# pk17r/online_3d_reconstruction

Measured on AMD Instinct MI355X. Metric: frames_per_sec, higher is better.
Workload: dtype f32; 1 GPU; synthetic 1280x720 dense stereo, jump_pixels 1, 200 frames/GPU, voxel_size 0.05, min_points_per_voxel 1, SOR off, frames resident in HBM (BASELINE.json configs[1]); frames_per_gpu=200, rows=720, cols=1280, jump_pixels=1, parallelism=frame-sharded x1

## Files before the change

### online_3d_reconstruction_amd/csrc/kernels/bookkeeping.inc

```

__global__ void k_minmax_init(float* mm, int64_t mm_stride, int slot, uint32_t* n_kp, int frames)
{
    const int i = blockIdx.x * blockDim.x + threadIdx.x;
    if (i < frames * 6) {
        const int f = i / 6, a = i % 6;
        mm[((int64_t)f * mm_stride + slot) * 6 + a] = (a < 3) ? __builtin_inff() : -__builtin_inff();
    }
    if (n_kp && i < frames) n_kp[i] = 0;
}
__global__ void k_set_counts(uint32_t* n_dev, uint32_t value, int frames)
{
    const int i = blockIdx.x * blockDim.x + threadIdx.x;
    if (i < frames) n_dev[i] = value;
}

__device__ __forceinline__ int64_t scan_row_len(const VoxelGeom* __restrict__ geom, int f, int pass, int n_tiles,
                                                int64_t L)
{
    if (!geom) return L;
    const VoxelGeom g = geom[f];
    if (g.overflow || pass >= (int)g.passes) return 0;
    return (int64_t)geom_bins(g) * n_tiles;
}
__device__ __forceinline__ int scan_live_tiles(const VoxelGeom* __restrict__ geom, int f, int n_tiles)
{
    if (!geom) return n_tiles;
    const int64_t live = ((int64_t)geom[f].n + kSortTile - 1) / kSortTile;
    return live < n_tiles ? (int)live : n_tiles;
}
__global__ __launch_bounds__(1024) void k_scan_rows(uint32_t* __restrict__ data, int64_t L_in, int64_t row_stride,
                                                    uint32_t* __restrict__ totals, const uint32_t* __restrict__ add,
                                                    const VoxelGeom* __restrict__ geom, int pass, int n_tiles,
                                                    int chunked)
{
    __shared__ uint32_t lds[1024 / 64 + 1];
    uint32_t* row = data + (int64_t)blockIdx.x * row_stride;
    int64_t L = scan_row_len(geom, blockIdx.x, pass, n_tiles, L_in);
    if (chunked) L = (L + 4095) / 4096;
    if (L == 0 && !totals) return;
    const int64_t chunk = (L + 1023) / 1024;
    const int64_t b = (int64_t)threadIdx.x * chunk;
    const int64_t e = (b + chunk < L) ? b + chunk : L;
    const bool tiles = geom != nullptr && !chunked;
    const int live = tiles ? scan_live_tiles(geom, blockIdx.x, n_tiles) : 0;
    uint32_t s = 0;
    {
        int t = tiles ? (int)(b % n_tiles) : 0;
        for (int64_t i = b; i < e; ++i) {
            if (!tiles || t < live) s += row[i];
            if (tiles && ++t == n_tiles) t = 0;
        }
    }
    uint32_t total;
    uint32_t run = block_excl_scan_u32<16>(s, lds, total);
    {
        int t = tiles ? (int)(b % n_tiles) : 0;
        for (int64_t i = b; i < e; ++i) {
            const uint32_t v = (!tiles || t < live) ? row[i] : 0u;
            row[i] = run;
            run += v;
            if (tiles && ++t == n_tiles) t = 0;
        }
    }
    if (totals && threadIdx.x == 0) totals[blockIdx.x] = total + (add ? add[blockIdx.x] : 0u);
}

__global__ __launch_bounds__(1024) void k_scan_hist_tm(uint32_t* __restrict__ hist, const VoxelGeom* __restrict__ geom, int pass,
                                                       int n_tiles, int all_live)
{
    extern __shared__ uint32_t tm_row[];
    __shared__ uint32_t lds[1024 / 64 + 1];
    const int f = blockIdx.x;
    const VoxelGeom g = geom[f];
// ... 24 lines not shown
            const uint32_t v = tm_row[t * (kMaxRadix + 1) + d];
            tm_row[t * (kMaxRadix + 1) + d] = run;
            run += v;
            if (++t == n_tiles) t = 0, ++d;
        }
    }
    __syncthreads();
    for (int i = threadIdx.x; i < words; i += 1024)
        if ((i & (kMaxRadix - 1)) < bins) row[i] = tm_row[(i >> kMaxRadixBits) * (kMaxRadix + 1) + (i & (kMaxRadix - 1))];
}

constexpr int kScanChunk = 4096;
__global__ __launch_bounds__(256) void k_scan_chunk_sums(const uint32_t* __restrict__ data, int64_t L_in,
                                                         int64_t row_stride, int n_chunks,
                                                         uint32_t* __restrict__ partial,
                                                         const VoxelGeom* __restrict__ geom, int pass, int n_tiles)
{
    __shared__ uint32_t lds[4];
    const int64_t L = scan_row_len(geom, blockIdx.y, pass, n_tiles, L_in);
    if ((int64_t)blockIdx.x * kScanChunk >= L) return;
    const uint32_t* row = data + (int64_t)blockIdx.y * row_stride;
    const int64_t b = (int64_t)blockIdx.x * kScanChunk + (int64_t)threadIdx.x * 16;
    const int live = scan_live_tiles(geom, blockIdx.y, n_tiles);
    int t = geom ? (int)(b % n_tiles) : 0;
    uint32_t s = 0;
#pragma unroll
    for (int k = 0; k < 16; ++k) {
        if (b + k < L && (!geom || t < live)) s += row[b + k];
        if (geom && ++t == n_tiles) t = 0;
    }
    s = wave_sum_u32(s);
    if ((threadIdx.x & 63) == 0) lds[threadIdx.x >> 6] = s;
    __syncthreads();
    if (threadIdx.x == 0) partial[(int64_t)blockIdx.y * n_chunks + blockIdx.x] = lds[0] + lds[1] + lds[2] + lds[3];
}
__global__ __launch_bounds__(256) void k_scan_chunk_apply(uint32_t* __restrict__ data, int64_t L_in, int64_t row_stride,
                                                          int n_chunks, const uint32_t* __restrict__ partial_scanned,
                                                          const VoxelGeom* __restrict__ geom, int pass, int n_tiles)
{
    __shared__ uint32_t lds[5];
    const int64_t L = scan_row_len(geom, blockIdx.y, pass, n_tiles, L_in);
    if ((int64_t)blockIdx.x * kScanChunk >= L) return;
    uint32_t* row = data + (int64_t)blockIdx.y * row_stride;
    const int64_t b = (int64_t)blockIdx.x * kScanChunk + (int64_t)threadIdx.x * 16;
    const int live = scan_live_tiles(geom, blockIdx.y, n_tiles);
    int t = geom ? (int)(b % n_tiles) : 0;
    uint32_t v[16];
    uint32_t s = 0;
#pragma unroll
    for (int k = 0; k < 16; ++k) {
        v[k] = (b + k < L && (!geom || t < live)) ? row[b + k] : 0u;
        s += v[k];
        if (geom && ++t == n_tiles) t = 0;
    }
    uint32_t total;
    uint32_t run = block_excl_scan_u32<4>(s, lds, total) + partial_scanned[(int64_t)blockIdx.y * n_chunks + blockIdx.x];
#pragma unroll
    for (int k = 0; k < 16; ++k) {
        if (b + k < L) row[b + k] = run;
        run += v[k];
    }
}

__global__ __launch_bounds__(kPtThreads) void k_points_minmax(const o3dr_point* __restrict__ in, int64_t in_fstride,
                                                              const uint32_t* __restrict__ n_dev, int64_t mm_stride,
                                                              float* __restrict__ mm)
// ... 26 lines not shown
```

### online_3d_reconstruction_amd/csrc/kernels/voxel_index.inc

```

__device__ __forceinline__ uint64_t geom_cells(const VoxelGeom& g)
{
    return (uint64_t)(uint32_t)g.div_b[0] * (uint64_t)(uint32_t)g.div_b[1] * (uint64_t)(uint32_t)g.div_b[2];
}
__device__ __forceinline__ void sort_plan(VoxelGeom& g, uint64_t cells)
{
    uint32_t nbits = 32;
    if (cells <= (1ull << 32)) nbits = cells > 1 ? 64u - (uint32_t)__clzll((long long)(cells - 1)) : 1u;
    if (nbits < 1) nbits = 1;
    g.passes = (nbits + kMaxRadixBits - 1) / kMaxRadixBits;
    g.bpp = (nbits + g.passes - 1) / g.passes;
}

__device__ __forceinline__ VoxelGeom voxel_geom_of(const float mn_in[3], const float mx_in[3], const float leaf[3], float z_offset,
                                                   uint32_t n)
{
    VoxelGeom g;
    g.n = n;
    g.overflow = 0;
    g.passes = 0;
    g.bpp = 1;
    g.buf0 = 0;
    g.grouped = 0;
    float mn[3], mx[3];
// ... 142 lines not shown
        if (lane == 0 && i > 0 && i < g.n) prev = group_coord_of(src[i - 1], g.inv, z_offset, cell);
        const bool head = i < g.n && (i == 0 || group_differs(gc, prev));
        c += head ? 1u : 0u;
        const unsigned long long hm = __ballot(head);
        if (lane < 16)
            head_bits[(int64_t)tile * 256 + k * 64 + (threadIdx.x >> 6) * 16 + lane] = (uint8_t)((hm >> (4 * lane)) & 15ull);
    }
    c = wave_sum_u32(c);
    if (lane == 0) lds[threadIdx.x >> 6] = c;
    __syncthreads();
    if (threadIdx.x == 0) seg_cnt[tile] = lds[0] + lds[1] + lds[2] + lds[3];
}
__global__ __launch_bounds__(256) void k_head_counts(const uint8_t* __restrict__ head_bits, const VoxelGeom* __restrict__ geom,
                                                     int n_tiles, uint32_t* __restrict__ seg_cnt)
{
    const int tile = blockIdx.x * 4 + (threadIdx.x >> 6), lane = threadIdx.x & 63;
    const VoxelGeom g = geom[0];
    if (g.overflow || tile >= n_tiles) return;
    const int64_t base = (int64_t)tile * kSegTile;
    uint32_t c = 0;
    if (base < g.n) {
        uint32_t bits = reinterpret_cast<const uint32_t*>(head_bits + (int64_t)tile * 256)[lane];
        const int64_t i0 = base + lane * 16;
#pragma unroll
        for (int q = 0; q < 16; ++q)
            if (i0 + q >= (int64_t)g.n) bits &= ~(1u << ((q >> 2) * 8 + (q & 3)));
        c = (uint32_t)__popc(bits & 0x0f0f0f0fu);
    }
    c = wave_sum_u32(c);
    if (lane == 0) seg_cnt[tile] = c;
}
```

### online_3d_reconstruction_amd/csrc/kernels/voxel_runs.inc

```



constexpr int kHeadWaves = 4;
__device__ __forceinline__ uint32_t run_heads_tile(const uint32_t* __restrict__ k, int f, int64_t cap, int64_t n, int tile, int lane)
{
    const int64_t i0 = (int64_t)tile * kSegTile + lane * 16;
    uint32_t kk[16];
    if (((((int64_t)f * cap) & 3) == 0) && i0 + 15 < n) {
#pragma unroll
        for (int q = 0; q < 4; ++q) {
            const uint4 v = *reinterpret_cast<const uint4*>(k + i0 + 4 * q);
            kk[4 * q] = v.x; kk[4 * q + 1] = v.y; kk[4 * q + 2] = v.z; kk[4 * q + 3] = v.w;
        }
    } else {
#pragma unroll
        for (int q = 0; q < 16; ++q) kk[q] = (i0 + q < n) ? k[i0 + q] : 0u;
    }
    uint32_t prev = (uint32_t)wave_shr1_i32((int32_t)kk[15]);
    if (lane == 0) prev = (i0 > 0 && i0 < n) ? k[i0 - 1] : 0u;
    uint32_t bits = 0;
#pragma unroll
    for (int q = 0; q < 16; ++q) {
        const int64_t i = i0 + q;
        if (i < n && (i == 0 || kk[q] != (q ? kk[q - 1] : prev))) bits |= 1u << ((q >> 2) * 8 + (q & 3));
// ... 145 lines not shown
}

__global__ __launch_bounds__(256) void k_frame_offsets(const VoxelGeom* __restrict__ geom, const uint32_t* __restrict__ n_vox,
                                                       const uint32_t* __restrict__ n_keep,
                                                       const uint32_t* __restrict__ n_grp, int frames, int passthrough,
                                                       uint32_t* __restrict__ n_out, uint64_t* __restrict__ out_off,
                                                       CloudCounters* __restrict__ cc, SortStats* __restrict__ stats,
                                                       const VoxelGeom* __restrict__ sort_geom, int side_heads)
{
    __shared__ uint32_t scan_lds[5];
    __shared__ unsigned long long acc[6];
    if (threadIdx.x < 6) acc[threadIdx.x] = 0;
    __syncthreads();
    const uint64_t base = cc->count;
    uint64_t carry = 0;
    for (int f0 = 0; f0 < frames; f0 += 256) {
        const int f = f0 + threadIdx.x;
        uint32_t m = 0;
        if (f < frames) {
            const VoxelGeom g = geom[f];
            if (passthrough) {
                m = g.n;
            } else if (g.overflow) {
                m = g.n;
                atomicOr(&acc[3], (unsigned long long)O3DR_STATUS_VOXEL_OVERFLOW);
            } else {
                m = (n_grp && sort_geom[f].grouped) ? n_grp[f] : (n_keep ? n_keep[f] : n_vox[f]);
                atomicAdd(&acc[0], (unsigned long long)sort_geom[f].n * g.passes);
                atomicAdd(&acc[5], (unsigned long long)sort_geom[f].n);
                if (side_heads && g.passes != 0u) atomicAdd(&acc[4], (unsigned long long)sort_geom[f].n);
                atomicAdd(&acc[1], (unsigned long long)g.n);
                atomicAdd(&acc[2], (unsigned long long)m);
            }
        }
        uint32_t total;
        const uint32_t excl = block_excl_scan_u32<4>(m, scan_lds, total);
        if (f < frames) {
            n_out[f] = m;
            out_off[f] = base + carry + excl;
        }
        carry += total;
    }
    __syncthreads();
    if (threadIdx.x == 0) {
        cc->count = base + carry;
        cc->status |= (uint32_t)acc[3];
        if (stats) {
            stats->sort_record_passes += acc[0];
            stats->voxel_points_in += acc[1];
            stats->voxel_points_out += acc[2];
            stats->sort_records += acc[5];
            stats->side_head_records += acc[4];
        }
    }
}

// ... 437 lines not shown
```

### online_3d_reconstruction_amd/csrc/o3dr_api.hip

```cpp
#include <dlfcn.h>
#include <stdio.h>
#include <stdlib.h>
#include <string.h>

#include <algorithm>
#include <cfloat>
#include <chrono>
#include <cmath>
#include <condition_variable>
#include <mutex>
#include <string>
#include <vector>

#include <rccl/rccl.h>

#include "../../include/o3dr_testing.h"
#include "o3dr_device.h"
#include "o3dr_image_stack.h"
#include "o3dr_profile.h"

using namespace o3dr;

static thread_local std::string g_err;
static int fail(int code, const char* what)
// ... 44 lines not shown
    Workspace ws;
    size_t ws_elems = 0;
    size_t ws_pts_elems = 0;
    int ws_frames = 0;
    size_t ws_emit_tiles = 0, ws_sort_tiles = 0, ws_seg_tiles = 0, ws_mm_floats = 0;
    DevBuf ws_block, ws_pts_block, ws_grid_block, ws_sor_block;
    int64_t ws_grid_cap = 0, ws_sor_cap = 0;
    int ws_grid_frames = 0, ws_sor_frames = 0;

    o3dr_point* cloud_big = nullptr;
    int64_t cloud_cap = 0;
    o3dr_point* cloud_alt = nullptr;
    int64_t cloud_alt_cap = 0;
    int64_t cloud_ub = 0;
    bool cloud_n_exact = true;
    float* cloud_box = nullptr;
    bool cloud_box_valid = false;
    uint32_t* cloud_heads = nullptr;
    int64_t cloud_heads_cap = 0;
    bool cloud_heads_valid = false;
    float cloud_heads_leaf[3] = {0.f, 0.f, 0.f};
    float cloud_heads_zo = 0.f;
    int cloud_box_enable = 1;
    CloudCounters* cc_big = nullptr;
    CloudCounters* cc_tmp = nullptr;
    CloudCounters* cc_host = nullptr;
    CloudCounters* cc_host_dev = nullptr;
    uint8_t* small_host = nullptr;
    uint32_t* n_host = nullptr;
    uint8_t* misc_dev = nullptr;
// ... 643 lines not shown
    }
    int zero(o3dr_ctx* c)
    {
        if (frames) HIPCHK(hipMemsetAsync(dev, 0, frames * words * sizeof(unsigned long long), c->stream));
        return O3DR_OK;
    }
    unsigned long long* of_frame(size_t f) const { return dev ? dev + f * words : nullptr; }
    int copy_back(o3dr_ctx* c)
    {
        host.resize(frames * words);
        if (frames) HIPCHK(hipMemcpyAsync(host.data(), dev, host.size() * sizeof(unsigned long long), hipMemcpyDeviceToHost, c->stream));
        return O3DR_OK;
    }
};

static int read_counters(o3dr_ctx* c, const CloudCounters* dev, CloudCounters* host, const CloudCounters* dev2 = nullptr,
                         CloudCounters* host2 = nullptr)
{
    HIPCHK(hipMemcpyAsync(c->cc_host, dev, sizeof(CloudCounters), hipMemcpyDeviceToHost, c->stream));
    if (dev2) HIPCHK(hipMemcpyAsync(c->cc_host + 1, dev2, sizeof(CloudCounters), hipMemcpyDeviceToHost, c->stream));
    HIPCHK(hipStreamSynchronize(c->stream));
    *host = *c->cc_host;
    if (dev2) {
        *host2 = c->cc_host[1];
        if (dev2 == c->cc_big) {
            c->cloud_ub = (int64_t)host2->count;
            c->cloud_n_exact = true;
        }
    }
    if (dev == c->cc_big) {
        c->cloud_ub = (int64_t)host->count;
        c->cloud_n_exact = true;
    }
    if ((host->status | (dev2 ? host2->status : 0u)) & O3DR_STATUS_INTERNAL)
        return fail(O3DR_ERR_INTERNAL, "a device-side gather guard tripped (record or point id outside its cloud); results are invalid");
    return O3DR_OK;
}

static int zero_counters(o3dr_ctx* c, CloudCounters* dev)
{
    HIPCHK(hipMemsetAsync(dev, 0, sizeof(CloudCounters), c->stream));
    return O3DR_OK;
}

static int bilateral_prepare(o3dr_ctx* c, int d, double sigma_color, double sigma_space)
{
    if (sigma_color <= 0) sigma_color = 1;
// ... 558 lines not shown
    for (int a = 0; a < 3; ++a) v.cloud_heads.inv[a] = 1.0f / leaf[a];
    v.cloud_heads.z_offset = zo;
}
static const uint8_t* heads_for_merge(o3dr_ctx* c, const float leaf[3], float zo)
{
    if (!c->cloud_heads_valid || !c->cloud_heads) return nullptr;
    if (leaf[0] != c->cloud_heads_leaf[0] || leaf[1] != c->cloud_heads_leaf[1] || leaf[2] != c->cloud_heads_leaf[2] ||
        zo != c->cloud_heads_zo)
        return nullptr;
    return reinterpret_cast<const uint8_t*>(c->cloud_heads);
}

extern "C" int o3dr_cloud_big_reset(o3dr_ctx* c)
{
    CTX_ENTER(c);
    ++c->cloud_gen;
    CHK(zero_counters(c, c->cc_big));
    CHK(cloud_box_clear(c));
    c->cloud_ub = 0;
    c->cloud_n_exact = true;
    return O3DR_OK;
}

extern "C" int o3dr_cloud_big_size(o3dr_ctx* c, int64_t* n, uint32_t* status)
{
    if (n) *n = 0;
    CTX_ENTER(c);
    CloudCounters cc;
    CHK(read_counters(c, c->cc_big, &cc));
    c->cloud_ub = (int64_t)cc.count;
    if (n) *n = (int64_t)cc.count;
    if (status) *status = cc.status;
    return O3DR_OK;
}

extern "C" int o3dr_cloud_big_read(o3dr_ctx* c, o3dr_point* out, int64_t out_capacity, int64_t* n_out, int32_t mem)
{
    if (n_out) *n_out = 0;
    CTX_ENTER(c);
    if (!n_out) return fail(O3DR_ERR_INVALID_ARG, "n_out is NULL");
    CloudCounters cc;
    CHK(read_counters(c, c->cc_big, &cc));
    const int64_t n = (int64_t)cc.count;
    if (n > out_capacity) return fail(O3DR_ERR_CAPACITY, "output buffer too small");
    if (n > 0) {
// ... 12 lines not shown
    if (n < 0 || (n > 0 && !pts)) return fail(O3DR_ERR_INVALID_ARG, "bad arguments");
    if (n == 0) return O3DR_OK;
    if (n >= (int64_t)0xffffffffLL) return fail(O3DR_ERR_INVALID_ARG, "more than 2^32-1 points in one append");
    CHK(cloud_make_room(c, n));
    const void* src;
    CHK(stage_in(c, c->st_in, pts, (size_t)n * sizeof(o3dr_point), mem, &src));
    CHK(ws_ensure(c, 1, 1, false));
    launch_set_counts(&c->prof, c->stream, c->ws.n_valid, (uint32_t)n, 1);
    const float unit_leaf[3] = {1.f, 1.f, 1.f};
    VoxelArgs v = voxel_args((const o3dr_point*)src, 0, c->ws.n_valid, 1, n, unit_leaf);
    v.out_base = c->cloud_big;
    v.cc = c->cc_big;
    v.passthrough = 1;
    c->cloud_box_valid = false;
    c->cloud_heads_valid = false;
    launch_voxel_grid(&c->prof, c->stream, c->ws, v);
    HIPCHK(hipGetLastError());
    c->cloud_ub += n;
    if (mem == O3DR_MEM_HOST) HIPCHK(hipStreamSynchronize(c->stream));
    return O3DR_OK;
}

extern "C" int o3dr_cloud_big_transform(o3dr_ctx* c, const float T[16])
{
    CTX_ENTER(c);
    if (!T) return fail(O3DR_ERR_INVALID_ARG, "T is NULL");
    CloudCounters cc;
    CHK(read_counters(c, c->cc_big, &cc));
    ++c->cloud_gen;
    launch_transform(&c->prof, c->stream, c->cloud_big, (int64_t)cc.count, T, c->cloud_big);
    HIPCHK(hipGetLastError());
    c->cloud_box_valid = false;
    c->cloud_heads_valid = false;
    return O3DR_OK;
}

static int accumulate_impl(o3dr_ctx* c, const uint8_t* disp, int64_t disp_frame_stride, int64_t disp_pitch,
                           const uint8_t* bgr, int64_t bgr_frame_stride, int64_t bgr_pitch, int32_t rows, int32_t cols,
                           const float* poses, int32_t n_frames, const float* kp_xy, const int64_t* kp_offsets, int32_t mem)
{
    CTX_ENTER(c);
    if (!c->has_Q) return fail(O3DR_ERR_NOT_CONFIGURED, "o3dr_set_camera has not been called");
    if (n_frames < 0 || (n_frames > 0 && !poses)) return fail(O3DR_ERR_INVALID_ARG, "bad frame list");
    if (mem != O3DR_MEM_HOST && mem != O3DR_MEM_DEVICE) return fail(O3DR_ERR_INVALID_ARG, "bad mem kind");
// ... 99 lines not shown
            launch_reproject(&c->prof, c->stream, a, nb, c->ws.pts, c->ws.tile_cnt, c->ws.n_kp, c->ws.n_valid, c->ws.mm,
                             c->ws.scan_partial);
        VoxelArgs v = voxel_args(c->ws.pts, cap, c->ws.n_valid, nb, cap, leaf, zo, mp);
        v.keys_ready = fused ? 1 : 0;
        v.emit_tiles = emit_tiles;
        v.cloud_box = c->cloud_box_valid ? c->cloud_box : nullptr;
        heads_for_append(c, v);
        v.out_base = c->cloud_big;
        v.cc = c->cc_big;
        v.passthrough = c->params.dont_downsample ? 1 : 0;
        v.mm_used = a.n_tiles + 1;
        v.stats = c->stats_dev;
        v.test_corrupt = c->test_corrupt;
        c->test_corrupt = 0;
        if (with_sor) CHK(sor_in_front(c, v, false));
        launch_voxel_grid(&c->prof, c->stream, c->ws, v);
        HIPCHK(hipGetLastError());
        c->cloud_ub += (int64_t)nb * cap;
        c->cloud_n_exact = false;
        if (streaming) HIPCHK(hipEventRecord(c->ev_done[slot], c->stream));
    }
    if (streaming) HIPCHK(hipStreamSynchronize(c->stream));
    return O3DR_OK;
}

extern "C" int o3dr_accumulate_frames(o3dr_ctx* c, const uint8_t* disp, int64_t disp_frame_stride, int64_t disp_pitch,
                                      const uint8_t* bgr, int64_t bgr_frame_stride, int64_t bgr_pitch, int32_t rows,
                                      int32_t cols, const float* poses, int32_t n_frames, int32_t mem)
{
    return accumulate_impl(c, disp, disp_frame_stride, disp_pitch, bgr, bgr_frame_stride, bgr_pitch, rows, cols, poses, n_frames,
// ... 346 lines not shown
    return O3DR_OK;
}
extern "C" int o3dr_cloud_big_recv_buffer(o3dr_ctx* c, int64_t n_points, void** ptr)
{
    CTX_ENTER(c);
    if (!ptr || n_points < 0) return fail(O3DR_ERR_INVALID_ARG, "bad arguments");
    CHK(alt_reserve(c, n_points > 0 ? n_points : 1));
    *ptr = c->cloud_alt;
    return O3DR_OK;
}
extern "C" int o3dr_cloud_big_adopt(o3dr_ctx* c, int64_t n_points)
{
    CTX_ENTER(c);
    if (n_points < 0 || n_points > c->cloud_alt_cap) return fail(O3DR_ERR_INVALID_ARG, "more points than the receive buffer holds");
    if (n_points >= (int64_t)0xffffffffLL) return fail(O3DR_ERR_INVALID_ARG, "cloud_big exceeds 2^32-1 points");
    ++c->cloud_gen;
    launch_set_cloud_count(c->stream, c->cc_big, (uint64_t)n_points);
    HIPCHK(hipGetLastError());
    swap_clouds(c);
    c->cloud_box_valid = false;
    c->cloud_heads_valid = false;
    c->cloud_ub = n_points;
    c->cloud_n_exact = true;
    return O3DR_OK;
}

extern "C" int o3dr_cloud_big_header_dev(o3dr_ctx* c, void* hdr_dev)
{
    CTX_ENTER(c);
    if (!hdr_dev) return fail(O3DR_ERR_INVALID_ARG, "hdr_dev is NULL");
    const float* box = c->cloud_box;
// ... 27 lines not shown

extern "C" int o3dr_cloud_big_partition_dev(o3dr_ctx* c, const void* hdrs_dev, int32_t n_hdrs, int32_t n_parts, int64_t* counts_dev)
{
    CTX_ENTER(c);
    if (!hdrs_dev || !counts_dev || n_hdrs < 1 || n_parts < 1 || n_parts > kMaxRadix)
        return fail(O3DR_ERR_INVALID_ARG, "bad arguments (1 <= n_parts <= 128)");
    HIPCHK(hipMemsetAsync(counts_dev, 0, sizeof(int64_t) * ((size_t)n_parts + 1), c->stream));
    const int64_t ub = c->cloud_ub;
    if (ub == 0 || !c->cloud_big) return O3DR_OK;
    if (ub >= (int64_t)0xffffffffLL) return fail(O3DR_ERR_INVALID_ARG, "cloud_big exceeds 2^32-1 points");
    CHK(ws_ensure(c, 1, ub, false));
    CHK(alt_reserve(c, ub));
    o3dr_point* nb = c->cloud_alt;
    launch_count_from_cc(c->stream, c->cc_big, c->ws.n_valid);
    const VoxelArgs v = slice_args(c, ub);
    ++c->cloud_gen;
    launch_partition(&c->prof, c->stream, c->ws, v, n_parts, nb, (uint64_t*)counts_dev, (uint32_t*)(counts_dev + n_parts), hdrs_dev, n_hdrs);
    if (hipGetLastError() != hipSuccess) return fail(O3DR_ERR_HIP, "partition launch failed");
    swap_clouds(c);
    c->cloud_heads_valid = false;
    return O3DR_OK;
}

extern "C" int o3dr_cloud_big_slice_counts_dev(o3dr_ctx* c, const void* hdrs_dev, int32_t n_hdrs, int32_t n_parts, int64_t* counts_dev)
{
    CTX_ENTER(c);
    if (!hdrs_dev || !counts_dev || n_hdrs < 1 || n_parts < 1 || n_parts > kMaxRadix)
        return fail(O3DR_ERR_INVALID_ARG, "bad arguments (1 <= n_parts <= 128)");
    c->place_ub = -1;
    HIPCHK(hipMemsetAsync(counts_dev, 0, sizeof(int64_t) * ((size_t)n_parts + 1), c->stream));
    const int64_t ub = c->cloud_ub;
// ... 20 lines not shown
    if (!counts || n_parts < 1 || n_parts > kMaxRadix || own_part < 0 || own_part >= n_parts || n_before < 0 || n_after < 0)
        return fail(O3DR_ERR_INVALID_ARG, "bad arguments");
    if (c->place_ub < 0 || c->place_parts != n_parts) return fail(O3DR_ERR_INVALID_ARG, "o3dr_cloud_big_slice_counts_dev must run first, for the same slices");
    int64_t n_local = 0;
    for (int p = 0; p < n_parts; ++p) {
        if (counts[p] < 0) return fail(O3DR_ERR_INVALID_ARG, "negative slice size");
        n_local += counts[p];
    }
    if (n_local > c->place_ub) return fail(O3DR_ERR_INVALID_ARG, "slice sizes above the cloud's size");
    const int64_t own = counts[own_part], send_start = n_before + own + n_after, total = send_start + (n_local - own);
    if (send_offset) *send_offset = send_start;
    const int64_t cap_counted = c->place_ub;
    c->place_ub = -1;
    if (n_before == 0 && n_after == 0 && own == n_local) return O3DR_OK;
    if (total >= (int64_t)0xffffffffLL) return fail(O3DR_ERR_INVALID_ARG, "the exchange buffer exceeds 2^32-1 points");
    ++c->cloud_gen;
    CHK(alt_reserve(c, total > 0 ? total : 1));
    int64_t* sh = (int64_t*)(c->misc_host + 2560);
    int64_t nat = 0, out_off = send_start;
    for (int p = 0; p < n_parts; ++p) {
        if (p == own_part) {
            sh[p] = n_before - nat;
        } else {
            sh[p] = out_off - nat;
            out_off += counts[p];
        }
        nat += counts[p];
    }
    HIPCHK(hipMemcpyAsync(c->misc_dev + 2560, sh, sizeof(int64_t) * (size_t)n_parts, hipMemcpyHostToDevice, c->stream));
    if (n_local > 0) {
        const VoxelArgs v = slice_args(c, cap_counted);
// ... 1 lines not shown
        if (hipGetLastError() != hipSuccess) return fail(O3DR_ERR_HIP, "slice placement launch failed");
    }
    swap_clouds(c);
    c->cloud_box_valid = false;
    c->cloud_heads_valid = false;
    c->cloud_ub = total;
    c->cloud_n_exact = false;
    return O3DR_OK;
}

extern "C" int o3dr_cloud_big_set_size(o3dr_ctx* c, int64_t n_points)
{
    CTX_ENTER(c);
    if (n_points < 0 || n_points > c->cloud_cap) return fail(O3DR_ERR_INVALID_ARG, "more points than the cloud buffer holds");
    if (n_points >= (int64_t)0xffffffffLL) return fail(O3DR_ERR_INVALID_ARG, "cloud_big exceeds 2^32-1 points");
    ++c->cloud_gen;
    launch_set_cloud_count(c->stream, c->cc_big, (uint64_t)n_points);
    HIPCHK(hipGetLastError());
    c->cloud_box_valid = false;
    c->cloud_heads_valid = false;
    c->cloud_ub = n_points;
    c->cloud_n_exact = true;
    return O3DR_OK;
}

extern "C" int o3dr_cloud_big_raw_view(o3dr_ctx* c, void** ptr, int64_t* capacity_points)
{
    CTX_ENTER(c);
    if (!ptr || !capacity_points) return fail(O3DR_ERR_INVALID_ARG, "ptr / capacity is NULL");
    *ptr = c->cloud_big;
    *capacity_points = c->cloud_cap;
// ... 38 lines not shown
    for (int p = 0; p < n_parts; ++p) counts[p] = 0;
    CloudCounters cc;
    CHK(read_counters(c, c->cc_big, &cc));
    const int64_t n = (int64_t)cc.count;
    c->cloud_ub = n;
    if (n == 0) return O3DR_OK;
    if (n >= (int64_t)0xffffffffLL) return fail(O3DR_ERR_INVALID_ARG, "cloud_big exceeds 2^32-1 points");
    CHK(ws_ensure(c, 1, n, false));
    CHK(alt_reserve(c, n));
    o3dr_point* nb = c->cloud_alt;
    launch_set_counts(&c->prof, c->stream, c->ws.n_valid, (uint32_t)n, 1);
    CHK(put_bbox(c, gmin, gmax));
    const VoxelArgs v = slice_args(c, n);
    uint32_t* ovf_dev = (uint32_t*)(c->misc_dev + 32);
    uint64_t* cnt_dev = (uint64_t*)(c->misc_dev + 64);
    ++c->cloud_gen;
    launch_partition(&c->prof, c->stream, c->ws, v, n_parts, nb, cnt_dev, ovf_dev);
    if (hipGetLastError() != hipSuccess) return fail(O3DR_ERR_HIP, "partition launch failed");
    HIPCHK(hipMemcpyAsync(c->misc_host, c->misc_dev, 64 + 8 * (size_t)n_parts, hipMemcpyDeviceToHost, c->stream));
    HIPCHK(hipStreamSynchronize(c->stream));
    swap_clouds(c);
    c->cloud_heads_valid = false;
    const uint32_t ovf = *(const uint32_t*)(c->misc_host + 32);
    const uint64_t* hc = (const uint64_t*)(c->misc_host + 64);
    for (int p = 0; p < n_parts; ++p) counts[p] = (int64_t)hc[p];
    if (status) *status = ovf ? O3DR_STATUS_VOXEL_OVERFLOW : 0u;
    return O3DR_OK;
}

struct RcclApi {
    void* handle = nullptr;
// ... 175 lines not shown
    if (own != O3DR_OK) {
        snprintf(buf, sizeof buf, "%s [every rank left the exchange]", own_msg.c_str());
        g_err = buf;
        return own;
    }
    snprintf(buf, sizeof buf, "rank %d failed with code %lld: every rank left the exchange together", first_rank, (long long)first_code);
    g_err = buf;
    return O3DR_ERR_PEER;
}

static int merge_partitioned_impl(o3dr_ctx* c, Transport& T, int32_t gather_result, o3dr_point* out, int64_t out_capacity,
                                  int64_t* n_out, int64_t* n_total, uint32_t* status, int32_t mem)
{
    const int W = T.W, rank = T.rank;
    if (W < 1 || W > kMaxRadix || rank < 0 || rank >= W) return fail(O3DR_ERR_INVALID_ARG, "communicators of 1..128 ranks are supported");
    ++c->cloud_gen;
    const size_t RW = (size_t)W + kRowExtra;
    const size_t o_hdr = 0, o_hdrs = 32, o_row = o_hdrs + 32 * (size_t)W, o_mat = o_row + 8 * RW;
    const size_t total_bytes = o_mat + 8 * (size_t)W * RW;
    CHK(dev_ensure(c, c->st_xchg, total_bytes));
    if (c->xchg_host_cap < total_bytes) {
        if (c->xchg_host) (void)hipHostFree(c->xchg_host);
        c->xchg_host = nullptr;
        c->xchg_host_cap = 0;
        if (hipHostMalloc((void**)&c->xchg_host, total_bytes, hipHostMallocDefault) != hipSuccess) return fail(O3DR_ERR_ALLOC, "hipHostMalloc failed");
        c->xchg_host_cap = total_bytes;
    }
    memset(c->xchg_stats, 0, sizeof c->xchg_stats);
    char* d = (char*)c->st_xchg.p;
    struct Hdr {
        float mn[3], mx[3];
// ... 3433 lines not shown
```

### online_3d_reconstruction_amd/csrc/o3dr_kernels.hip

```cpp
#include <string.h>

#include "o3dr_device.h"
#include "o3dr_profile.h"

namespace o3dr {

#include "kernels/util.inc"
#include "kernels/reproject.inc"
#include "kernels/bookkeeping.inc"
#include "kernels/prepass.inc"
#include "kernels/voxel_index.inc"
#include "kernels/radix_sort.inc"
#include "kernels/voxel_runs.inc"
#include "kernels/incremental.inc"
#include "kernels/multigpu.inc"
#include "kernels/sor.inc"
#include "kernels/small.inc"
#include "kernels/rigid_core.inc"
#include "kernels/nn.inc"
#include "kernels/mls.inc"
#include "kernels/cluster.inc"
#include "kernels/cell_order.inc"
#include "kernels/plane.inc"
#include "kernels/mesh.inc"
// ... 4 lines not shown
#include "kernels/plane_disparity.inc"
#include "kernels/orb.inc"
#include "kernels/stereo.inc"
#include "kernels/disparity_filter.inc"
#include "kernels/multiview.inc"
#include "kernels/segment_image.inc"
#include "kernels/rectify.inc"
#include "kernels/pose_chain.inc"
#include "kernels/ransac.inc"
#include "kernels/pose_graph.inc"

static inline int cdiv64(int64_t a, int64_t b) { return (int)((a + b - 1) / b); }

static void launch_scan(hipStream_t s, uint32_t* data, int64_t L, int64_t row_stride, int frames, uint32_t* totals,
                        const uint32_t* add, uint32_t* partial, const VoxelGeom* geom = nullptr, int pass = 0,
                        int n_tiles = 0)
{
    if (L <= 4 * kScanChunk) {
        k_scan_rows<<<frames, 1024, 0, s>>>(data, L, row_stride, totals, add, geom, pass, n_tiles, 0);
        return;
    }
    const int n_chunks = cdiv64(L, kScanChunk);
    k_scan_chunk_sums<<<dim3(n_chunks, frames), 256, 0, s>>>(data, L, row_stride, n_chunks, partial, geom, pass, n_tiles);
    k_scan_rows<<<frames, 1024, 0, s>>>(partial, L, n_chunks, totals, add, geom, pass, n_tiles, 1);
    k_scan_chunk_apply<<<dim3(n_chunks, frames), 256, 0, s>>>(data, L, row_stride, n_chunks, partial, geom, pass, n_tiles);
}

void launch_minmax_init(Profiler* pf, hipStream_t s, float* mm, int64_t mm_stride, int slot, uint32_t* n_kp, int frames)
{
    ProfScope ps(pf, O3DR_K_OTHER, s);
    k_minmax_init<<<cdiv64(frames * 6, 256), 256, 0, s>>>(mm, mm_stride, slot, n_kp, frames);
}

void launch_set_counts(Profiler* pf, hipStream_t s, uint32_t* n_dev, uint32_t value, int frames)
{
    ProfScope ps(pf, O3DR_K_OTHER, s);
    k_set_counts<<<cdiv64(frames, 256), 256, 0, s>>>(n_dev, value, frames);
}

void launch_small_frame(Profiler* pf, hipStream_t s, const ReprojectArgs& a, const float* kp_xy, int n_kp, int downsample,
// ... 139 lines not shown
}

static void group_run_front(Profiler* pf, hipStream_t s, Workspace& ws, const SortShape& sh, const o3dr_point* in, float z_offset,
                            const uint8_t* rec_heads, int64_t shift_first, int64_t shift_n, int force_runs, int64_t grp_slots)
{
    const int F = sh.frames, n_seg_tiles = sh.n_seg_tiles;
    const uint8_t* hb = rec_heads && shift_n <= 0 ? rec_heads : ws.head_bits;
    {
        ProfScope ps(pf, O3DR_K_KEYGEN, s);
        if (rec_heads && shift_n > 0) {
            const int64_t bytes = (int64_t)n_seg_tiles * 256;
            k_inc_heads_shift<<<cdiv64(bytes, 256), 256, 0, s>>>(rec_heads, (uint64_t)shift_first, (uint64_t)shift_n, ws.head_bits,
                                                                 (uint64_t)bytes);
        }
        if (rec_heads)
            k_head_counts<<<cdiv64(n_seg_tiles, 4), 256, 0, s>>>(hb, ws.geom, n_seg_tiles, ws.seg_cnt);
        else
            k_group_heads<<<n_seg_tiles, 256, 0, s>>>(in, ws.geom, z_offset, n_seg_tiles, ws.seg_cnt, ws.head_bits);
    }
    {
        ProfScope ps(pf, O3DR_K_OTHER, s);
        launch_scan(s, ws.seg_cnt, n_seg_tiles, n_seg_tiles, F, ws.n_runs, nullptr, ws.scan_partial);
    }
    {
        ProfScope ps(pf, O3DR_K_SEGMENT, s);
        k_run_geom<<<cdiv64(F, 64), 64, 0, s>>>(ws.geom, ws.n_runs, F, ws.geom_runs, force_runs, grp_slots);
        k_run_starts<<<dim3(cdiv64(n_seg_tiles, kStartWaves), F), kStartWaves * kWave, 0, s>>>(
            ws.keys[0], ws.keys[1], sh.cap, ws.geom, n_seg_tiles, ws.seg_cnt, ws.n_runs, ws.run_start, 0, ws.keys[1], ws.geom_runs, in,
            z_offset, hb);
    }
}
// ... 140 lines not shown
            {
                ProfScope ps(pf, O3DR_K_OTHER, s);
                launch_scan(s, ws.seg_cnt, n_seg_tiles, n_seg_tiles, F, ws.n_out, nullptr, ws.scan_partial);
            }
            {
                ProfScope ps(pf, O3DR_K_SEGMENT, s);
                k_keep_write<<<sgrid, 256, 0, s>>>(ws.seg_start, cap, sort_geom, ws.n_vox, v.min_points, n_seg_tiles, ws.seg_cnt,
                                                  ws.keep_idx);
            }
            n_keep = ws.n_out;
        }
        if (v.test_corrupt) corrupt_payload(s, ws, sort_geom);
    }
    if (cap > 0 && use_runs) {
        {
            ProfScope ps(pf, O3DR_K_OTHER, s);
            (void)hipMemsetAsync(ws.grp_cnt, 0, sizeof(uint32_t) * (size_t)(max_groups + 1), s);
        }
        {
            ProfScope ps(pf, O3DR_K_CENTROID_RUNS, s);
            int64_t nwg = cdiv64(max_groups < cap ? max_groups : cap, kGroupWaves);
            if (nwg > 16384) nwg = 16384;
            if (nwg < 1) nwg = 1;
            k_centroid_groups<<<(int)nwg, kGroupWaves * kWave, 0, s>>>(
                v.in, ws.keys[0], ws.keys[1], ws.vals[0], ws.vals[1], ws.seg_start, ws.run_start, ws.geom_runs, ws.geom, ws.n_vox,
                v.z_offset, v.min_points, reinterpret_cast<uint4*>(ws.pts), grp_slots, ws.grp_cnt, v.cc);
        }
        {
            ProfScope ps(pf, O3DR_K_OTHER, s);
            launch_scan(s, ws.grp_cnt, max_groups + 1, max_groups + 1, 1, ws.n_grp_out, nullptr, ws.scan_partial);
        }
    }
    {
        ProfScope ps(pf, O3DR_K_OTHER, s);
        k_frame_offsets<<<1, 256, 0, s>>>(ws.geom, ws.n_vox, n_keep, use_runs ? ws.n_grp_out : nullptr, F, v.passthrough,
                                          ws.n_out, ws.out_off, v.cc, v.stats, sort_geom,
                                          (!use_runs && ws.side && !v.passthrough && cap > 0) ? 1 : 0);
    }
    const int nbx = cdiv64(cap, kPtThreads);
    if (cap > 0 && use_runs) {
        ProfScope ps(pf, O3DR_K_CENTROID_RUNS, s);
        int64_t nwg = cdiv64(cap, 256);
        if (nwg > 8192) nwg = 8192;
        k_group_compact<<<(int)nwg, 256, 0, s>>>(v.in, ws.geom_runs, ws.geom, ws.n_vox, ws.grp_cnt,
                                                reinterpret_cast<const uint4*>(ws.pts), ws.out_off, v.z_offset, v.out_base);
// ... 841 lines not shown
```

Measured before the change: 36040 frames/s.

## Bound group-count scan by live length, drop memset, densify head counts, cache size

The group-count scan now takes a per-frame live length (n_vox), so it scans only live+1 entries and treats the rest as zero. This lets the grp_cnt memset be removed, relying on the centroid kernel to write every live slot. k_head_counts now handles four tiles per wave using 16-byte loads and a 16-lane shuffle reduction, and k_frame_offsets reduces its stat atomics across each wave before issuing them. The host cloud-size query reuses the last read counters instead of doing a device read while the cloud is unchanged. The risk is stale grp_cnt entries if any live slot goes unwritten, and a stale cached size if some write path misses the invalidation.

After: 36450 frames/s (median of 6 runs). 1.1% higher.

```diff
diff --git a/online_3d_reconstruction_amd/csrc/kernels/bookkeeping.inc b/online_3d_reconstruction_amd/csrc/kernels/bookkeeping.inc
--- a/online_3d_reconstruction_amd/csrc/kernels/bookkeeping.inc
+++ b/online_3d_reconstruction_amd/csrc/kernels/bookkeeping.inc
@@ -15,8 +15,9 @@
 }
 
 __device__ __forceinline__ int64_t scan_row_len(const VoxelGeom* __restrict__ geom, int f, int pass, int n_tiles,
-                                                int64_t L)
+                                                int64_t L, const uint32_t* __restrict__ live = nullptr)
 {
+    if (live) return (int64_t)live[f] + 1 < L ? (int64_t)live[f] + 1 : L;
     if (!geom) return L;
     const VoxelGeom g = geom[f];
     if (g.overflow || pass >= (int)g.passes) return 0;
@@ -31,23 +32,24 @@
 __global__ __launch_bounds__(1024) void k_scan_rows(uint32_t* __restrict__ data, int64_t L_in, int64_t row_stride,
                                                     uint32_t* __restrict__ totals, const uint32_t* __restrict__ add,
                                                     const VoxelGeom* __restrict__ geom, int pass, int n_tiles,
-                                                    int chunked)
+                                                    int chunked, const uint32_t* __restrict__ live)
 {
     __shared__ uint32_t lds[1024 / 64 + 1];
     uint32_t* row = data + (int64_t)blockIdx.x * row_stride;
-    int64_t L = scan_row_len(geom, blockIdx.x, pass, n_tiles, L_in);
+    int64_t L = scan_row_len(geom, blockIdx.x, pass, n_tiles, L_in, live);
+    const int64_t Lr = (live && !chunked) ? L - 1 : (chunked ? (L + 4095) / 4096 : L);
     if (chunked) L = (L + 4095) / 4096;
     if (L == 0 && !totals) return;
     const int64_t chunk = (L + 1023) / 1024;
     const int64_t b = (int64_t)threadIdx.x * chunk;
     const int64_t e = (b + chunk < L) ? b + chunk : L;
     const bool tiles = geom != nullptr && !chunked;
-    const int live = tiles ? scan_live_tiles(geom, blockIdx.x, n_tiles) : 0;
+    const int live_tiles = tiles ? scan_live_tiles(geom, blockIdx.x, n_tiles) : 0;
     uint32_t s = 0;
     {
         int t = tiles ? (int)(b % n_tiles) : 0;
         for (int64_t i = b; i < e; ++i) {
-            if (!tiles || t < live) s += row[i];
+            if (i < Lr && (!tiles || t < live_tiles)) s += row[i];
             if (tiles && ++t == n_tiles) t = 0;
         }
     }
@@ -56,7 +58,7 @@
     {
         int t = tiles ? (int)(b % n_tiles) : 0;
         for (int64_t i = b; i < e; ++i) {
-            const uint32_t v = (!tiles || t < live) ? row[i] : 0u;
+            const uint32_t v = (i < Lr && (!tiles || t < live_tiles)) ? row[i] : 0u;
             row[i] = run;
             run += v;
             if (tiles && ++t == n_tiles) t = 0;
@@ -111,11 +113,13 @@
 __global__ __launch_bounds__(256) void k_scan_chunk_sums(const uint32_t* __restrict__ data, int64_t L_in,
                                                          int64_t row_stride, int n_chunks,
                                                          uint32_t* __restrict__ partial,
-                                                         const VoxelGeom* __restrict__ geom, int pass, int n_tiles)
+                                                         const VoxelGeom* __restrict__ geom, int pass, int n_tiles,
+                                                         const uint32_t* __restrict__ live_len)
 {
     __shared__ uint32_t lds[4];
-    const int64_t L = scan_row_len(geom, blockIdx.y, pass, n_tiles, L_in);
+    const int64_t L = scan_row_len(geom, blockIdx.y, pass, n_tiles, L_in, live_len);
     if ((int64_t)blockIdx.x * kScanChunk >= L) return;
+    const int64_t Lr = live_len ? L - 1 : L;
     const uint32_t* row = data + (int64_t)blockIdx.y * row_stride;
     const int64_t b = (int64_t)blockIdx.x * kScanChunk + (int64_t)threadIdx.x * 16;
     const int live = scan_live_tiles(geom, blockIdx.y, n_tiles);
@@ -123,7 +127,7 @@
     uint32_t s = 0;
 #pragma unroll
     for (int k = 0; k < 16; ++k) {
-        if (b + k < L && (!geom || t < live)) s += row[b + k];
+        if (b + k < Lr && (!geom || t < live)) s += row[b + k];
         if (geom && ++t == n_tiles) t = 0;
     }
     s = wave_sum_u32(s);
@@ -133,11 +137,13 @@
 }
 __global__ __launch_bounds__(256) void k_scan_chunk_apply(uint32_t* __restrict__ data, int64_t L_in, int64_t row_stride,
                                                           int n_chunks, const uint32_t* __restrict__ partial_scanned,
-                                                          const VoxelGeom* __restrict__ geom, int pass, int n_tiles)
+                                                          const VoxelGeom* __restrict__ geom, int pass, int n_tiles,
+                                                          const uint32_t* __restrict__ live_len)
 {
     __shared__ uint32_t lds[5];
-    const int64_t L = scan_row_len(geom, blockIdx.y, pass, n_tiles, L_in);
+    const int64_t L = scan_row_len(geom, blockIdx.y, pass, n_tiles, L_in, live_len);
     if ((int64_t)blockIdx.x * kScanChunk >= L) return;
+    const int64_t Lr = live_len ? L - 1 : L;
     uint32_t* row = data + (int64_t)blockIdx.y * row_stride;
     const int64_t b = (int64_t)blockIdx.x * kScanChunk + (int64_t)threadIdx.x * 16;
     const int live = scan_live_tiles(geom, blockIdx.y, n_tiles);
@@ -146,7 +152,7 @@
     uint32_t s = 0;
 #pragma unroll
     for (int k = 0; k < 16; ++k) {
-        v[k] = (b + k < L && (!geom || t < live)) ? row[b + k] : 0u;
+        v[k] = (b + k < Lr && (!geom || t < live)) ? row[b + k] : 0u;
         s += v[k];
         if (geom && ++t == n_tiles) t = 0;
     }
diff --git a/online_3d_reconstruction_amd/csrc/kernels/voxel_index.inc b/online_3d_reconstruction_amd/csrc/kernels/voxel_index.inc
--- a/online_3d_reconstruction_amd/csrc/kernels/voxel_index.inc
+++ b/online_3d_reconstruction_amd/csrc/kernels/voxel_index.inc
@@ -180,19 +180,29 @@
 __global__ __launch_bounds__(256) void k_head_counts(const uint8_t* __restrict__ head_bits, const VoxelGeom* __restrict__ geom,
                                                      int n_tiles, uint32_t* __restrict__ seg_cnt)
 {
-    const int tile = blockIdx.x * 4 + (threadIdx.x >> 6), lane = threadIdx.x & 63;
+    static_assert(kSegTile == 16 * 64, "16 lanes of 64 records per segment tile");
+    const int lane = threadIdx.x & 63, sub = lane & 15;
+    const int tile = (blockIdx.x * 4 + (threadIdx.x >> 6)) * 4 + (lane >> 4);
     const VoxelGeom g = geom[0];
-    if (g.overflow || tile >= n_tiles) return;
-    const int64_t base = (int64_t)tile * kSegTile;
+    if (g.overflow) return;
+    const int64_t n = g.n;
+    const int64_t i0 = (int64_t)tile * kSegTile + sub * 64;
     uint32_t c = 0;
-    if (base < g.n) {
-        uint32_t bits = reinterpret_cast<const uint32_t*>(head_bits + (int64_t)tile * 256)[lane];
-        const int64_t i0 = base + lane * 16;
-#pragma unroll
-        for (int q = 0; q < 16; ++q)
-            if (i0 + q >= (int64_t)g.n) bits &= ~(1u << ((q >> 2) * 8 + (q & 3)));
-        c = (uint32_t)__popc(bits & 0x0f0f0f0fu);
-    }
-    c = wave_sum_u32(c);
-    if (lane == 0) seg_cnt[tile] = c;
-}
+    if (tile < n_tiles && i0 < n) {
+        const uint4 v = *reinterpret_cast<const uint4*>(head_bits + (int64_t)tile * 256 + sub * 16);
+        uint32_t w4[4] = {v.x, v.y, v.z, v.w};
+#pragma unroll
+        for (int k = 0; k < 4; ++k) {
+            const int64_t i = i0 + 16 * k;
+            if (i + 16 > n) {
+#pragma unroll
+                for (int q = 0; q < 16; ++q)
+                    if (i + q >= n) w4[k] &= ~(1u << ((q >> 2) * 8 + (q & 3)));
+            }
+            c += (uint32_t)__popc(w4[k] & 0x0f0f0f0fu);
+        }
+    }
+#pragma unroll
+    for (int m = 8; m >= 1; m >>= 1) c += (uint32_t)__shfl_xor((int)c, m, 64);
+    if (sub == 0 && tile < n_tiles) seg_cnt[tile] = c;
+}
diff --git a/online_3d_reconstruction_amd/csrc/kernels/voxel_runs.inc b/online_3d_reconstruction_amd/csrc/kernels/voxel_runs.inc
--- a/online_3d_reconstruction_amd/csrc/kernels/voxel_runs.inc
+++ b/online_3d_reconstruction_amd/csrc/kernels/voxel_runs.inc
@@ -183,6 +183,7 @@
     __syncthreads();
     const uint64_t base = cc->count;
     uint64_t carry = 0;
+    unsigned long long mine[6] = {0ull, 0ull, 0ull, 0ull, 0ull, 0ull};
     for (int f0 = 0; f0 < frames; f0 += 256) {
         const int f = f0 + threadIdx.x;
         uint32_t m = 0;
@@ -192,14 +193,15 @@
                 m = g.n;
             } else if (g.overflow) {
                 m = g.n;
-                atomicOr(&acc[3], (unsigned long long)O3DR_STATUS_VOXEL_OVERFLOW);
+                mine[3] |= (unsigned long long)O3DR_STATUS_VOXEL_OVERFLOW;
             } else {
+                const uint32_t n_rec = sort_geom[f].n;
                 m = (n_grp && sort_geom[f].grouped) ? n_grp[f] : (n_keep ? n_keep[f] : n_vox[f]);
-                atomicAdd(&acc[0], (unsigned long long)sort_geom[f].n * g.passes);
-                atomicAdd(&acc[5], (unsigned long long)sort_geom[f].n);
-                if (side_heads && g.passes != 0u) atomicAdd(&acc[4], (unsigned long long)sort_geom[f].n);
-                atomicAdd(&acc[1], (unsigned long long)g.n);
-                atomicAdd(&acc[2], (unsigned long long)m);
+                mine[0] += (unsigned long long)n_rec * g.passes;
+                mine[5] += (unsigned long long)n_rec;
+                if (side_heads && g.passes != 0u) mine[4] += (unsigned long long)n_rec;
+                mine[1] += (unsigned long long)g.n;
+                mine[2] += (unsigned long long)m;
             }
         }
         uint32_t total;
@@ -209,6 +211,21 @@
             out_off[f] = base + carry + excl;
         }
         carry += total;
+    }
+#pragma unroll
+    for (int a = 0; a < 6; ++a) {
+        unsigned long long v = mine[a];
+#pragma unroll
+        for (int msk = 32; msk >= 1; msk >>= 1) {
+            const unsigned long long o = __shfl_xor(v, msk, 64);
+            v = a == 3 ? (v | o) : (v + o);
+        }
+        if ((threadIdx.x & 63) == 0 && v != 0ull) {
+            if (a == 3)
+                atomicOr(&acc[a], v);
+            else
+                atomicAdd(&acc[a], v);
+        }
     }
     __syncthreads();
     if (threadIdx.x == 0) {
diff --git a/online_3d_reconstruction_amd/csrc/o3dr_api.hip b/online_3d_reconstruction_amd/csrc/o3dr_api.hip
--- a/online_3d_reconstruction_amd/csrc/o3dr_api.hip
+++ b/online_3d_reconstruction_amd/csrc/o3dr_api.hip
@@ -82,6 +82,8 @@
     int64_t cloud_alt_cap = 0;
     int64_t cloud_ub = 0;
     bool cloud_n_exact = true;
+    bool size_seen = false;
+    uint32_t size_status = 0;
     float* cloud_box = nullptr;
     bool cloud_box_valid = false;
     uint32_t* cloud_heads = nullptr;
@@ -755,6 +757,12 @@
     }
 };
 
+static inline void cloud_appended(o3dr_ctx* c) { c->size_seen = false; }
+static inline void cloud_written(o3dr_ctx* c)
+{
+    ++c->cloud_gen;
+    c->size_seen = false;
+}
 static int read_counters(o3dr_ctx* c, const CloudCounters* dev, CloudCounters* host, const CloudCounters* dev2 = nullptr,
                          CloudCounters* host2 = nullptr)
 {
@@ -767,11 +775,15 @@
         if (dev2 == c->cc_big) {
             c->cloud_ub = (int64_t)host2->count;
             c->cloud_n_exact = true;
+            c->size_status = host2->status;
+            c->size_seen = true;
         }
     }
     if (dev == c->cc_big) {
         c->cloud_ub = (int64_t)host->count;
         c->cloud_n_exact = true;
+        c->size_status = host->status;
+        c->size_seen = true;
     }
     if ((host->status | (dev2 ? host2->status : 0u)) & O3DR_STATUS_INTERNAL)
         return fail(O3DR_ERR_INTERNAL, "a device-side gather guard tripped (record or point id outside its cloud); results are invalid");
@@ -1360,7 +1372,7 @@
 extern "C" int o3dr_cloud_big_reset(o3dr_ctx* c)
 {
     CTX_ENTER(c);
-    ++c->cloud_gen;
+    cloud_written(c);
     CHK(zero_counters(c, c->cc_big));
     CHK(cloud_box_clear(c));
     c->cloud_ub = 0;
@@ -1373,8 +1385,14 @@
     if (n) *n = 0;
     CTX_ENTER(c);
     CloudCounters cc;
-    CHK(read_counters(c, c->cc_big, &cc));
-    c->cloud_ub = (int64_t)cc.count;
+    if (c->size_seen && c->cloud_n_exact) {
+        cc.count = (uint64_t)c->cloud_ub;
+        cc.status = c->size_status;
+        if (cc.status & O3DR_STATUS_INTERNAL)
+            return fail(O3DR_ERR_INTERNAL, "a device-side gather guard tripped (record or point id outside its cloud); results are invalid");
+    } else {
+        CHK(read_counters(c, c->cc_big, &cc));
+    }
     if (n) *n = (int64_t)cc.count;
     if (status) *status = cc.status;
     return O3DR_OK;
@@ -1417,6 +1435,7 @@
     v.passthrough = 1;
     c->cloud_box_valid = false;
     c->cloud_heads_valid = false;
+    cloud_appended(c);
     launch_voxel_grid(&c->prof, c->stream, c->ws, v);
     HIPCHK(hipGetLastError());
     c->cloud_ub += n;
@@ -1430,7 +1449,7 @@
     if (!T) return fail(O3DR_ERR_INVALID_ARG, "T is NULL");
     CloudCounters cc;
     CHK(read_counters(c, c->cc_big, &cc));
-    ++c->cloud_gen;
+    cloud_written(c);
     launch_transform(&c->prof, c->stream, c->cloud_big, (int64_t)cc.count, T, c->cloud_big);
     HIPCHK(hipGetLastError());
     c->cloud_box_valid = false;
@@ -1560,6 +1579,7 @@
         v.test_corrupt = c->test_corrupt;
         c->test_corrupt = 0;
         if (with_sor) CHK(sor_in_front(c, v, false));
+        cloud_appended(c);
         launch_voxel_grid(&c->prof, c->stream, c->ws, v);
         HIPCHK(hipGetLastError());
         c->cloud_ub += (int64_t)nb * cap;
@@ -1936,7 +1956,7 @@
     CTX_ENTER(c);
     if (n_points < 0 || n_points > c->cloud_alt_cap) return fail(O3DR_ERR_INVALID_ARG, "more points than the receive buffer holds");
     if (n_points >= (int64_t)0xffffffffLL) return fail(O3DR_ERR_INVALID_ARG, "cloud_big exceeds 2^32-1 points");
-    ++c->cloud_gen;
+    cloud_written(c);
     launch_set_cloud_count(c->stream, c->cc_big, (uint64_t)n_points);
     HIPCHK(hipGetLastError());
     swap_clouds(c);
@@ -1994,7 +2014,7 @@
     o3dr_point* nb = c->cloud_alt;
     launch_count_from_cc(c->stream, c->cc_big, c->ws.n_valid);
     const VoxelArgs v = slice_args(c, ub);
-    ++c->cloud_gen;
+    cloud_written(c);
     launch_partition(&c->prof, c->stream, c->ws, v, n_parts, nb, (uint64_t*)counts_dev, (uint32_t*)(counts_dev + n_parts), hdrs_dev, n_hdrs);
     if (hipGetLastError() != hipSuccess) return fail(O3DR_ERR_HIP, "partition launch failed");
     swap_clouds(c);
@@ -2045,7 +2065,7 @@
     c->place_ub = -1;
     if (n_before == 0 && n_after == 0 && own == n_local) return O3DR_OK;
     if (total >= (int64_t)0xffffffffLL) return fail(O3DR_ERR_INVALID_ARG, "the exchange buffer exceeds 2^32-1 points");
-    ++c->cloud_gen;
+    cloud_written(c);
     CHK(alt_reserve(c, total > 0 ? total : 1));
     int64_t* sh = (int64_t*)(c->misc_host + 2560);
     int64_t nat = 0, out_off = send_start;
@@ -2077,7 +2097,7 @@
     CTX_ENTER(c);
     if (n_points < 0 || n_points > c->cloud_cap) return fail(O3DR_ERR_INVALID_ARG, "more points than the cloud buffer holds");
     if (n_points >= (int64_t)0xffffffffLL) return fail(O3DR_ERR_INVALID_ARG, "cloud_big exceeds 2^32-1 points");
-    ++c->cloud_gen;
+    cloud_written(c);
     launch_set_cloud_count(c->stream, c->cc_big, (uint64_t)n_points);
     HIPCHK(hipGetLastError());
     c->cloud_box_valid = false;
@@ -2146,7 +2166,7 @@
     const VoxelArgs v = slice_args(c, n);
     uint32_t* ovf_dev = (uint32_t*)(c->misc_dev + 32);
     uint64_t* cnt_dev = (uint64_t*)(c->misc_dev + 64);
-    ++c->cloud_gen;
+    cloud_written(c);
     launch_partition(&c->prof, c->stream, c->ws, v, n_parts, nb, cnt_dev, ovf_dev);
     if (hipGetLastError() != hipSuccess) return fail(O3DR_ERR_HIP, "partition launch failed");
     HIPCHK(hipMemcpyAsync(c->misc_host, c->misc_dev, 64 + 8 * (size_t)n_parts, hipMemcpyDeviceToHost, c->stream));
@@ -2352,7 +2372,7 @@
 {
     const int W = T.W, rank = T.rank;
     if (W < 1 || W > kMaxRadix || rank < 0 || rank >= W) return fail(O3DR_ERR_INVALID_ARG, "communicators of 1..128 ranks are supported");
-    ++c->cloud_gen;
+    cloud_written(c);
     const size_t RW = (size_t)W + kRowExtra;
     const size_t o_hdr = 0, o_hdrs = 32, o_row = o_hdrs + 32 * (size_t)W, o_mat = o_row + 8 * RW;
     const size_t total_bytes = o_mat + 8 * (size_t)W * RW;
diff --git a/online_3d_reconstruction_amd/csrc/o3dr_kernels.hip b/online_3d_reconstruction_amd/csrc/o3dr_kernels.hip
--- a/online_3d_reconstruction_amd/csrc/o3dr_kernels.hip
+++ b/online_3d_reconstruction_amd/csrc/o3dr_kernels.hip
@@ -42,16 +42,16 @@
 
 static void launch_scan(hipStream_t s, uint32_t* data, int64_t L, int64_t row_stride, int frames, uint32_t* totals,
                         const uint32_t* add, uint32_t* partial, const VoxelGeom* geom = nullptr, int pass = 0,
-                        int n_tiles = 0)
+                        int n_tiles = 0, const uint32_t* live = nullptr)
 {
     if (L <= 4 * kScanChunk) {
-        k_scan_rows<<<frames, 1024, 0, s>>>(data, L, row_stride, totals, add, geom, pass, n_tiles, 0);
+        k_scan_rows<<<frames, 1024, 0, s>>>(data, L, row_stride, totals, add, geom, pass, n_tiles, 0, live);
         return;
     }
     const int n_chunks = cdiv64(L, kScanChunk);
-    k_scan_chunk_sums<<<dim3(n_chunks, frames), 256, 0, s>>>(data, L, row_stride, n_chunks, partial, geom, pass, n_tiles);
-    k_scan_rows<<<frames, 1024, 0, s>>>(partial, L, n_chunks, totals, add, geom, pass, n_tiles, 1);
-    k_scan_chunk_apply<<<dim3(n_chunks, frames), 256, 0, s>>>(data, L, row_stride, n_chunks, partial, geom, pass, n_tiles);
+    k_scan_chunk_sums<<<dim3(n_chunks, frames), 256, 0, s>>>(data, L, row_stride, n_chunks, partial, geom, pass, n_tiles, live);
+    k_scan_rows<<<frames, 1024, 0, s>>>(partial, L, n_chunks, totals, add, geom, pass, n_tiles, 1, live);
+    k_scan_chunk_apply<<<dim3(n_chunks, frames), 256, 0, s>>>(data, L, row_stride, n_chunks, partial, geom, pass, n_tiles, live);
 }
 
 void launch_minmax_init(Profiler* pf, hipStream_t s, float* mm, int64_t mm_stride, int slot, uint32_t* n_kp, int frames)
@@ -221,7 +221,7 @@
                                                                  (uint64_t)bytes);
         }
         if (rec_heads)
-            k_head_counts<<<cdiv64(n_seg_tiles, 4), 256, 0, s>>>(hb, ws.geom, n_seg_tiles, ws.seg_cnt);
+            k_head_counts<<<cdiv64(n_seg_tiles, 16), 256, 0, s>>>(hb, ws.geom, n_seg_tiles, ws.seg_cnt);
         else
             k_group_heads<<<n_seg_tiles, 256, 0, s>>>(in, ws.geom, z_offset, n_seg_tiles, ws.seg_cnt, ws.head_bits);
     }
@@ -392,10 +392,6 @@
     }
     if (cap > 0 && use_runs) {
         {
-            ProfScope ps(pf, O3DR_K_OTHER, s);
-            (void)hipMemsetAsync(ws.grp_cnt, 0, sizeof(uint32_t) * (size_t)(max_groups + 1), s);
-        }
-        {
             ProfScope ps(pf, O3DR_K_CENTROID_RUNS, s);
             int64_t nwg = cdiv64(max_groups < cap ? max_groups : cap, kGroupWaves);
             if (nwg > 16384) nwg = 16384;
@@ -406,7 +402,7 @@
         }
         {
             ProfScope ps(pf, O3DR_K_OTHER, s);
-            launch_scan(s, ws.grp_cnt, max_groups + 1, max_groups + 1, 1, ws.n_grp_out, nullptr, ws.scan_partial);
+            launch_scan(s, ws.grp_cnt, max_groups + 1, max_groups + 1, 1, ws.n_grp_out, nullptr, ws.scan_partial, nullptr, 0, 0, ws.n_vox);
         }
     }
     {
```
